# grantjr1842/delayed-streams-modeling

Hardware: AMD Instinct MI355X
Metric: real-time stream throughput, stt-1b-en_fr @ bs=64 per GPU (Mimi encode + LM decode per 80 ms frame) (higher is better)
Workload: dtype bf16 weights + bf16 KV, f32 activations as three exact bf16 pieces, f32 accumulate (v_mfma_f32_16x16x32_bf16); 1 GPU; stt-1b-en_fr batch=64 streaming, ring KV cache full (750 frames), Mimi encode + LM decode HIP path; streams_per_gpu=64, parallelism=replicas x1 (independent stream batches, no per-step collective), streams=encoder stream || 2 LM group stream(s)

## Files before the change

### delayed-streams-modeling_amd/__init__.py

```python
import ctypes as C
import os
import numpy as np

_HERE = os.path.dirname(os.path.abspath(__file__))
LIB_PATH = os.path.join(_HERE, "libdsm_mi355x.so")

FRAME_SIZE = 1920
MAX_RATIOS = 8
MAX_EXTRA_HEADS = 8


class TransformerConfig(C.Structure):
    _fields_ = [(n, C.c_int) for n in (
        "d_model", "num_heads", "num_layers", "dim_feedforward", "context", "max_period",
        "gating", "norm", "positional_embedding", "layer_scale", "conv_layout")]


class MimiConfig(C.Structure):
    _fields_ = [
        ("channels", C.c_int), ("dimension", C.c_int), ("n_filters", C.c_int),
        ("n_residual_layers", C.c_int), ("n_ratios", C.c_int), ("ratios", C.c_int * MAX_RATIOS),
        ("kernel_size", C.c_int), ("residual_kernel_size", C.c_int), ("last_kernel_size", C.c_int),
        ("dilation_base", C.c_int), ("compress", C.c_int), ("transformer", TransformerConfig),
        ("quantizer_n_q", C.c_int), ("quantizer_bins", C.c_int), ("quantizer_dim", C.c_int),
# ... 62 lines not shown
    _fields_ = [("self", C.c_void_p), ("batch_size", C.c_int), ("asr_delay_in_tokens", C.c_int),
                ("extra_heads_num", C.c_int), ("encode_step", BE_ENCODE), ("reset_slot", BE_RESET),
                ("step_tokens", BE_STEP), ("poll_msgs", BE_POLL), ("last_error", BE_ERROR),
                ("encode_async", BE_ENCODE_ASYNC), ("step_ticket", BE_STEP_TICKET)]


class Metrics(C.Structure):
    _fields_ = [("last_encode_us", C.c_double), ("last_lm_us", C.c_double),
                ("algorithmic_bytes_encode", C.c_double), ("algorithmic_bytes_lm", C.c_double),
                ("steps_encode", C.c_uint64), ("steps_lm", C.c_uint64),
                ("graph_launches", C.c_uint64), ("eager_bodies", C.c_uint64),
                ("capture_failures", C.c_uint64), ("capture_error", C.c_char * 96)]


MSG_STEP, MSG_WORD, MSG_END_WORD = 0, 1, 2

ABI_SYMBOLS = [
    "dsm_mimi_config_v0_1", "dsm_asr_config_stt_1b_en_fr", "dsm_asr_config_stt_2_6b_en",
    "dsm_asr_create", "dsm_asr_create_from_arena", "dsm_asr_weight_arena", "dsm_destroy", "dsm_last_error", "dsm_mimi_encode_step", "dsm_asr_step_tokens",
    "dsm_asr_step_pcm", "dsm_asr_poll_msgs", "dsm_asr_reset_slot", "dsm_mimi_reset_slot", "dsm_sync",
    "dsm_get_metrics", "dsm_batch_size", "dsm_n_q", "dsm_mimi_encode_step_dev", "dsm_asr_step_tokens_dev",
    "dsm_streams_join", "dsm_debug_read", "dsm_debug_gemm_plan", "dsm_asr_step_pcm_dev", "dsm_prof_enable", "dsm_prof_read",
    "dsm_asr_create_replica", "dsm_asr_set_seed", "dsm_debug_set_positions", "dsm_debug_set_text_tokens", "dsm_mimi_decode_step", "dsm_mimi_decode_step_dev",
    "dsm_lm_stream_groups", "dsm_debug_serialize_groups", "dsm_prof_read_device", "dsm_prof_timeline", "dsm_prof_timeline_read",
    "dsm_wav_decode", "dsm_mp3_decode", "dsm_mp3_decode_info", "dsm_mp3_probe", "dsm_resample", "dsm_pcm_decode",
    "dsm_mp3_test_synth", "dsm_mp3_test_tables", "dsm_mp3_test_imdct", "dsm_free", "dsm_linear_resampler_new", "dsm_linear_resampler_process",
    "dsm_linear_resampler_free", "dsm_ogg_demux_new", "dsm_ogg_demux_free", "dsm_ogg_demux_push", "dsm_ogg_demux_next",
    "dsm_ogg_demux_info", "dsm_worker_set_opus_decoder", "dsm_ogg_mux_new", "dsm_ogg_mux_free", "dsm_ogg_mux_header", "dsm_ogg_mux_page",
    "dsm_inmsg_encode", "dsm_outmsg_encode", "dsm_inmsg_decode", "dsm_outmsg_decode", "dsm_worker_create",
    "dsm_worker_create_with_backend", "dsm_worker_destroy", "dsm_worker_last_error", "dsm_worker_set_detokenizer", "dsm_worker_open", "dsm_worker_close",
    "dsm_worker_send", "dsm_worker_send_body", "dsm_worker_step", "dsm_worker_step_encode", "dsm_worker_step_model",
    "dsm_mimi_encode_step_async", "dsm_asr_step_tokens_ticket", "dsm_worker_recv", "dsm_worker_buffered",
    "dsm_tts_config_v202501", "dsm_tts_create", "dsm_tts_destroy", "dsm_tts_last_error", "dsm_tts_step",
    "dsm_tts_audio_tokens", "dsm_tts_step_idx", "dsm_tts_reset_slot", "dsm_tts_debug_read", "dsm_tts_get_metrics", "dsm_tts_set_sampling",
    "dsm_tts_set_ca_src", "dsm_tts_attach_mimi", "dsm_tts_step_pcm", "dsm_tts_recv_pcm", "dsm_tts_pcm_pending",
    "dsm_tts_attach_speaker_encoder", "dsm_tts_encode_voice", "dsm_tts_speaker_empty",
]
PROF_TAGS = ["attn_lm", "gemm_lm", "attn_mimi", "gemm_mimi", "rvq", "other"]

_lib = None


def load_library(path=None):
    global _lib
    if _lib is not None and path is None:
        return _lib
    p = path or LIB_PATH
# ... 34 lines not shown
    lib.dsm_mimi_decode_step_dev.argtypes = [vp, vp, vp, vp]
    lib.dsm_mimi_decode_step_dev.restype = C.c_int
    lib.dsm_debug_set_positions.argtypes = [vp, C.c_uint32, C.c_uint32]
    lib.dsm_debug_set_positions.restype = C.c_int
    lib.dsm_asr_create_replica.argtypes = [vp, vp, C.c_int, C.c_int, C.POINTER(vp)]
    lib.dsm_asr_create_replica.restype = C.c_int
    lib.dsm_asr_set_seed.argtypes = [vp, C.c_int, C.c_uint64]
    lib.dsm_asr_set_seed.restype = C.c_int
    lib.dsm_debug_set_text_tokens.argtypes = [vp, vp]
    lib.dsm_debug_set_text_tokens.restype = C.c_int
    lib.dsm_prof_enable.argtypes = [vp, C.c_uint]
    lib.dsm_prof_read.argtypes = [vp, C.POINTER(C.c_double), C.POINTER(C.c_uint64)]
    for name in ("dsm_mimi_encode_step", "dsm_asr_step_tokens", "dsm_asr_step_pcm", "dsm_asr_poll_msgs",
                 "dsm_asr_reset_slot", "dsm_mimi_reset_slot", "dsm_sync", "dsm_get_metrics", "dsm_batch_size",
                 "dsm_n_q", "dsm_mimi_encode_step_dev", "dsm_asr_step_tokens_dev", "dsm_streams_join",
                 "dsm_debug_read", "dsm_asr_step_pcm_dev", "dsm_prof_enable", "dsm_prof_read"):
        getattr(lib, name).restype = C.c_int
    lib.dsm_prof_read_device.argtypes = [vp, C.POINTER(C.c_double), C.POINTER(C.c_uint64)]
    lib.dsm_prof_read_device.restype = C.c_int
    lib.dsm_lm_stream_groups.argtypes = [vp, C.POINTER(C.c_int), C.POINTER(C.c_int), C.c_int]
    lib.dsm_lm_stream_groups.restype = C.c_int
    lib.dsm_debug_serialize_groups.argtypes = [vp, C.c_int]
    lib.dsm_debug_serialize_groups.restype = C.c_int
    lib.dsm_debug_gemm_plan.argtypes = [C.c_int] * 9 + [C.c_char_p, C.c_size_t]
    lib.dsm_debug_gemm_plan.restype = C.c_int
    lib.dsm_wav_decode.argtypes = [C.c_char_p, C.c_size_t, C.POINTER(C.POINTER(C.c_float)), C.POINTER(C.c_size_t),
                                   C.POINTER(C.c_int)]
    lib.dsm_wav_decode.restype = C.c_int
    for name in ("dsm_mp3_decode", "dsm_pcm_decode"):
        getattr(lib, name).argtypes = lib.dsm_wav_decode.argtypes
        getattr(lib, name).restype = C.c_int
    lib.dsm_mp3_decode_info.argtypes = [C.c_char_p, C.c_size_t, C.POINTER(C.POINTER(C.c_float)), C.POINTER(C.c_size_t), C.POINTER(Mp3Info)]
    lib.dsm_mp3_decode_info.restype = C.c_int
    lib.dsm_mp3_probe.argtypes = [C.c_char_p, C.c_size_t, C.POINTER(Mp3Info)]
    lib.dsm_mp3_probe.restype = C.c_int
    lib.dsm_resample.argtypes = [C.c_void_p, C.c_size_t, C.c_int, C.c_int, C.POINTER(C.POINTER(C.c_float)), C.POINTER(C.c_size_t)]
    lib.dsm_resample.restype = C.c_int
    lib.dsm_mp3_test_synth.argtypes = [C.c_void_p, C.c_int, C.c_void_p]
    lib.dsm_mp3_test_tables.argtypes = [C.c_int, C.POINTER(C.c_int), C.POINTER(C.c_int), C.c_void_p, C.c_void_p, C.c_int]
    lib.dsm_mp3_test_imdct.argtypes = [C.c_void_p, C.c_int, C.c_void_p]
    lib.dsm_free.argtypes = [vp]
    lib.dsm_free.restype = None
    lib.dsm_linear_resampler_new.argtypes = [C.c_uint32, C.c_uint32]
    lib.dsm_linear_resampler_new.restype = vp
    lib.dsm_linear_resampler_process.argtypes = [vp, vp, C.c_size_t, vp, C.c_size_t]
    lib.dsm_linear_resampler_process.restype = C.c_size_t
# ... 553 lines not shown
    def prof_read_device(self):
        tot = (C.c_double * len(PROF_TAGS))()
        cnt = (C.c_uint64 * len(PROF_TAGS))()
        self._check(self.lib.dsm_prof_read_device(self.h, tot, cnt))
        return {t: (tot[i], cnt[i]) for i, t in enumerate(PROF_TAGS)}

    def prof_timeline(self, on):
        self._check(self.lib.dsm_prof_timeline(self.h, 1 if on else 0))

    def prof_timeline_read(self, cap=1 << 16):
        sid, kind, tag = (C.c_int * cap)(), (C.c_int * cap)(), (C.c_int * cap)()
        t0, t1 = (C.c_double * cap)(), (C.c_double * cap)()
        n = self._check(self.lib.dsm_prof_timeline_read(self.h, sid, kind, tag, t0, t1, cap))
        return [(sid[i], kind[i], PROF_TAGS[tag[i]], t0[i], t1[i]) for i in range(n)]

    def stream_groups(self):
        a, b = (C.c_int * 8)(), (C.c_int * 8)()
        g = self._check(self.lib.dsm_lm_stream_groups(self.h, a, b, 8))
        return [(a[i], b[i]) for i in range(g)]

    def debug_serialize_groups(self, on):
        self._check(self.lib.dsm_debug_serialize_groups(self.h, 1 if on else 0))

    def prof_enable(self, tags):
        mask = 0
        for t in tags:
            mask |= 1 << PROF_TAGS.index(t)
        self._check(self.lib.dsm_prof_enable(self.h, mask))

    def prof_read(self):
        tot = (C.c_double * len(PROF_TAGS))()
        cnt = (C.c_uint64 * len(PROF_TAGS))()
        self._check(self.lib.dsm_prof_read(self.h, tot, cnt))
        return {t: (tot[i], cnt[i]) for i, t in enumerate(PROF_TAGS)}


class TtsEngine:

    def __init__(self, cfg, batch_size, lm_path, device_id=0):
        self.lib = load_library()
        self.cfg, self.B, self.S = cfg, batch_size, cfg.dep_num_slices
        self.n_speakers = 0
        h = C.c_void_p()
        rc = self.lib.dsm_tts_create(C.byref(cfg), device_id, batch_size, lm_path.encode(), C.byref(h))
        if rc != 0:
            msg = self.lib.dsm_tts_last_error(None)
# ... 104 lines not shown
```

### delayed-streams-modeling_amd/csrc/dsm_engine.hip

```cpp
#include <hip/hip_runtime.h>

#include <cmath>
#include <cstdarg>
#include <cstdio>
#include <cstdlib>
#include <cstring>
#include <atomic>
#include <mutex>
#include <shared_mutex>
#include <string>
#include <set>
#include <vector>

#include "../../include/dsm.h"
#include "dsm_device.h"
#include "dsm_config_presets.h"
#include "dsm_gemm_plan.h"
#include "dsm_kernels.h"
#include "dsm_numerics.h"
#include "dsm_safetensors.h"

static thread_local std::string g_create_error;

static int dsm_env_int(const char* name, int dflt) {
// ... 172 lines not shown
  TransformerState tr;
  struct Group {
    int b0 = 0, nb = 0;
    TransformerState view;
  };
  std::vector<Group> groups;
};

struct HostItem {
  size_t step_idx = 0;
  std::vector<uint32_t> word_tokens;
  bool unended_word = false;
  double last_stop_time = 0.0;
};

}

struct dsm_engine : DsmDevice {
  dsm_asr_config cfg{};
  int B = 0;
  hipEvent_t ev_grp_in[kMaxGroups] = {}, ev_stagger[kMaxGroups] = {};
  bool grp_busy = false;
  bool serialize_groups = false;
  hipEvent_t ev_codes_consumed = nullptr;
  bool codes_consumed_valid = false;
  hipEvent_t ev_join = nullptr, ev_a = nullptr, ev_b = nullptr, ev_c = nullptr, ev_d = nullptr;
  MimiW mimi_w;
  MimiState mimi[2];
  std::atomic<bool> mimi1_ready{false};
  std::mutex mimi1_mu;
  MimiDecState dec;
  LmW lm_w;
  LmState lm;
  GraphSlot *g_enc[2] = {}, *g_grp[kMaxGroups] = {};
  float* h_pcm = nullptr;
  float* h_pcm1 = nullptr;
  uint8_t* h_mask = nullptr;
  uint32_t *h_codes = nullptr, *h_text = nullptr;
  float* h_prs = nullptr;
  std::vector<HostItem> items;
  size_t model_step_idx = 0;
  std::vector<dsm_asr_msg> msgs;
  std::vector<uint32_t> msg_tokens;
  dsm_metrics metrics{};
  static constexpr int kPipe = 4;
  struct PipeSlot {
// ... 534 lines not shown
    case GEMM_BX3_LOOP: hipLaunchKernelGGL((gemm_bx3_kernel<KVT, MT, NT, EPI, true>), grid, block, p.lds, st, a); break;
    case GEMM_BX3_LOOP_NT2:
      if constexpr (MT == 4)
        hipLaunchKernelGGL((gemm_bx3_kernel<KVT, 4, (NT == 1 ? 2 : NT), (EPI == EPI_GATE ? EPI_STORE : EPI), true>), grid, block, p.lds, st, a);
      break;
    case GEMM_BX3_SPLIT:
      if constexpr (MT == 4) hipLaunchKernelGGL((gemm_bx3_kernel<KVT, 4, NT, EPI, false>), grid, block, p.lds, st, a);
      break;
    case GEMM_BX3U_2:
      if constexpr (MT == 2) hipLaunchKernelGGL((gemm_bx3u_kernel<KVT, 2, NT, EPI, 8, 0, 4>), grid, block, p.lds, st, a);
      break;
    case GEMM_BX3U_1:
      if constexpr (MT == 1) hipLaunchKernelGGL((gemm_bx3u_kernel<KVT, 1, NT, EPI, 8>), grid, block, p.lds, st, a);
      break;
    case GEMM_WK:
      if constexpr (MT == 1 && EPI == EPI_GATE && NT == 2)
        hipLaunchKernelGGL((gemm_wk_kernel<KVT, 1, 2, EPI_GATE, 1, 4, 2, true, 4>), grid, block, p.lds, st, a);
      break;
    case GEMM_NO_FIT: break;
  }
}

template <typename WT, typename KVT, int EPI, int NT>
int launch_gemm(DsmDevice* e, hipStream_t st, const GemmArgs& args, bool aligned, Slabs* slabs = nullptr) {
  static_assert(EPI_STORE == GEMM_EPI_STORE && EPI_QKV == GEMM_EPI_QKV && EPI_GATE == GEMM_EPI_GATE && EPI_RVQ == GEMM_EPI_RVQ, "");
  static_assert(LoopDepth<uint16_t, 1>::MAX == 4 && LoopDepth<uint16_t, 2>::MAX == 2 && LoopDepth<float, 1>::MAX == 2, "plan_gemm's `deep`");
  auto ok4 = [](const RowMap& m) { return m.ld % 4 == 0 && m.bstride % 4 == 0; };
  GemmQuery q;
  q.weight_bf16 = sizeof(WT) == 2;
  q.epi = EPI;
  q.NT = NT;
  q.M = args.M; q.N = args.N; q.K = args.K; q.Kpad = args.Kpad;
  q.nt_stride = args.nt_stride;
  q.aligned = aligned;
  q.has_Y = args.Y != nullptr; q.has_Y2 = args.Y2 != nullptr; q.has_res = args.res != nullptr;
  q.has_bias = args.bias != nullptr; q.has_norm = args.norm_out != nullptr;
  q.y_ok4 = ok4(args.ymap); q.y2_ok4 = ok4(args.y2map); q.res_ok4 = ok4(args.rmap);
  q.y_bstride0 = args.ymap.bstride == 0;
  q.may_defer = slabs != nullptr;
  GemmKnobs k;
  k.dot_mode = e->dot_mode;
  k.chunk_loop_min_tiles = e->chunk_loop_min_tiles;
  k.smallk_min_tiles = e->smallk_min_tiles;
  k.smallk_mt = e->smallk_mt;
  k.loop_depth = e->loop_depth;
  const GemmPlan p = plan_gemm(q, k);
  if (p.form == GEMM_NO_FIT) {
    e->set_error("GEMM K=%d: chunk partials do not fit in LDS", args.K);
    return DSM_ERR_INVALID;
  }
  GemmArgs a = args;
  a.vec = p.vec;
  a.chunk_loop = p.chunk_loop;
  a.wg_cols = p.wg_cols;
  a.nt_stride = p.nt_stride;
  a.ws_ntiles = p.ws_ntiles;
  const int sid = e->sid(st);
  if (p.ws_bytes) {
    if (p.ws_bytes > e->gemm_ws_cap[sid]) {
      if (e->capturing) {
        e->capture_failed = true;
        e->set_error("split-K workspace grew during a graph capture");
        return DSM_ERR_STATE;
      }
      e->ws_gen += 1;
      HIPCHK(hipStreamSynchronize(st));
      if (e->gemm_ws[sid]) HIPCHK(hipFree(e->gemm_ws[sid]));
      e->gemm_ws[sid] = nullptr;
      e->gemm_ws_cap[sid] = 0;
      void* ws = nullptr;
      HIPCHK(hipMalloc(&ws, p.ws_bytes));
      e->gemm_ws[sid] = reinterpret_cast<float*>(ws);
      e->gemm_ws_cap[sid] = p.ws_bytes;
    }
    a.ws = e->gemm_ws[sid];
  }
  if (p.tiled) a.ts = e->timeline ? e->dev_ts_slot(e->tag_gemm[sid], sid, 1, 2) : nullptr;
  const int ph = e->prof_begin(e->tag_gemm[sid], st);
  switch (p.MT) {
    case 4: launch_form<WT, KVT, EPI, NT, 4>(p, st, a); break;
    case 2: launch_form<WT, KVT, EPI, NT, 2>(p, st, a); break;
    default: launch_form<WT, KVT, EPI, NT, 1>(p, st, a); break;
  }
  switch (p.reduce) {
    case GEMM_RED_NONE: case GEMM_RED_CONSUMER: break;
    case GEMM_RED_ROWS1: hipLaunchKernelGGL(gemm_reduce_rows_kernel<1>, dim3(a.M), dim3(256), 0, st, a, p.chunks); break;
    case GEMM_RED_ROWS2: hipLaunchKernelGGL(gemm_reduce_rows_kernel<2>, dim3(a.M), dim3(512), 0, st, a, p.chunks); break;
    case GEMM_RED_ROWS4: hipLaunchKernelGGL(gemm_reduce_rows_kernel<4>, dim3(a.M), dim3(1024), 0, st, a, p.chunks); break;
    case GEMM_RED_TILES: {
      const int out_tiles = ((a.M + 15) / 16) * ((a.N + 15) / 16);
      hipLaunchKernelGGL((gemm_reduce_kernel<KVT, EPI>), dim3((out_tiles + 3) / 4), dim3(256), 0, st, a, p.chunks);
      break;
    }
  }
  e->prof_end(ph, st);
  HIPCHK(hipGetLastError());
  if (p.row_norm) {
    hipLaunchKernelGGL(row_norm_kernel, dim3(a.M), dim3(256), 0, st, a.norm_out, a.Y, a.norm_w, a.norm_b, a.M,
                       a.N, a.norm_eps, a.norm_rms);
    HIPCHK(hipGetLastError());
  }
  if (slabs) {
    *slabs = Slabs{};
// ... 90 lines not shown
  a.xmap = xmap;
  a.W = L.w;
  a.wpacked = L.packed ? 1 : 0;
  a.Kpad = L.Kpad;
  a.K = L.K;
  a.N = L.N;
  a.M = M;
  a.nt_stride = 16;
  a.bias = L.bias;
  return a;
}

float norm_eps(int rms) { return rms ? 1e-8f : 1e-5f; }

void set_norm(GemmArgs& a, const float* w, const float* b, float* out, int rms) {
  a.norm_w = w;
  a.norm_b = b;
  a.norm_out = out;
  a.norm_eps = norm_eps(rms);
  a.norm_rms = rms;
}

template <typename WT>
int gemm_store(DsmDevice* e, hipStream_t st, const GemmArgs& a, bool aligned = true, Slabs* slabs = nullptr) {
  return launch_gemm<WT, float, EPI_STORE, 1>(e, st, a, aligned, slabs);
}

int run_conv(DsmDevice* e, hipStream_t st, const ConvGeom& c, const float* cat, int B, float* y, RowMap ymap,
             float* y2, RowMap y2map, const float* res, RowMap rmap) {
  const long bstride = (long)(c.S + c.T_in) * c.in_c;
  GemmArgs a = base_args(c.lin, cat, batch_map(bstride, c.T_out, c.stride * c.in_c, 0), B * c.T_out);
  a.Y = y;
  a.ymap = ymap;
  a.Y2 = y2;
  a.y2map = y2map;
  a.res = res;
  a.rmap = rmap;
  bool aligned = ((c.stride * c.in_c) % 4 == 0) && (bstride % 4 == 0);
  return gemm_store<float>(e, st, a, aligned);
}

}

#include "dsm_engine_api.inc"
#include "dsm_tts.inc"
#include "dsm_speaker.inc"
#include "dsm_audio.inc"
#include "dsm_worker.inc"
```

### delayed-streams-modeling_amd/csrc/dsm_engine_api.inc

```

namespace {

template <typename KVT, int HD, int T>
int launch_attn_t(DsmDevice* e, hipStream_t st, float* out, const float* q, const void* k, const void* v,
                  const uint32_t* start_pos, const uint8_t* active, int B, int H, int ctx, int d, const AttnFused& fq) {
  constexpr int UNR = (sizeof(KVT) == 2 && T == 1 && HD == 128) ? 8 : 4;
  size_t lds = sizeof(float) * ((size_t)T * ctx + 4 * T * HD + 16);
  if ((long)B * H >= 2048 && (size_t)2 * ctx * HD * sizeof(KVT) >= (size_t)256 * 1024) lds += e->attn_lds_pad;
  if (lds > 64 * 1024) {
    static size_t allowed = 0;
    if (lds > allowed) {
      HIPCHK(hipFuncSetAttribute(reinterpret_cast<const void*>(&attn_kernel<KVT, HD, T, UNR>), hipFuncAttributeMaxDynamicSharedMemorySize, (int)lds));
      allowed = lds;
    }
  }
  const int tag = e->tag_attn[e->sid(st)];
  if (T == 1 && HD == 64 && ctx <= 32) {
    const int ph = e->prof_begin(tag, st);
    hipLaunchKernelGGL((attn_small_kernel<KVT, 64>), dim3((B * H + 3) / 4), dim3(256), 0, st, out, q, reinterpret_cast<const KVT*>(k),
                       reinterpret_cast<const KVT*>(v), start_pos, active, B * H, H, ctx, d, fq);
    e->prof_end(ph, st);
    HIPCHK(hipGetLastError());
    return 0;
  }
// ... 132 lines not shown

int fork_groups(DsmDevice* e, hipStream_t st, size_t G) {
  if (G > 1) {
    HIPCHK(hipEventRecord(e->ev_fork, st));
    for (size_t g = 1; g < G; ++g) HIPCHK(hipStreamWaitEvent(e->s_grp[g], e->ev_fork, 0));
  }
  return 0;
}
template <typename F>
int run_groups(DsmDevice* e, hipStream_t st, size_t G, bool serialize, F&& body) {
  for (size_t g = G; g-- > 0;) {
    hipStream_t gs = (g == 0 || serialize) ? st : e->s_grp[g];
    if (int rc = body(g, gs)) return rc;
    if (g > 0) HIPCHK(hipEventRecord(e->ev_grp_done[g], gs));
  }
  return 0;
}
int join_groups(DsmDevice* e, hipStream_t st, size_t G) {
  for (size_t g = 1; g < G; ++g) HIPCHK(hipStreamWaitEvent(st, e->ev_grp_done[g], 0));
  return 0;
}

int seanet_encode(DsmDevice* e, hipStream_t st, const MimiW& w, SeanetEnc& s, const float* cat_init, int B, int r, float* out,
                  RowMap omap, bool front_done = false) {
  const RowMap none = plain_map(1, 1);
  const size_t n = w.stages.size();
  const ConvGeom g0 = over_frames(w.init_conv, r), gf = over_frames(w.final_conv, r);
  if (!front_done)
    if (int rc = run_conv(e, st, g0, cat_init, B, s.stages[0].y, plain_map(B * g0.T_out, g0.out_c), s.stages[0].cat_ra,
                          cat_map(over_frames(w.stages[0].ra, r)), nullptr, none))
      return rc;
  for (size_t i = 0; i < n; ++i) {
    const ConvGeom ra = over_frames(w.stages[i].ra, r), rb = over_frames(w.stages[i].rb, r), dn = over_frames(w.stages[i].down, r);
    SeanetEnc::Stage& ss = s.stages[i];
    if (!(i == 0 && front_done)) {
      if (int rc = run_conv(e, st, ra, ss.cat_ra, B, nullptr, none, ss.cat_rb, cat_map(rb), nullptr, none)) return rc;
      if (int rc = run_conv(e, st, rb, ss.cat_rb, B, nullptr, none, ss.cat_down, cat_map(dn), ss.y, plain_map(B * rb.T_out, rb.out_c)))
        return rc;
    }
    if (i + 1 < n) {
      if (int rc = run_conv(e, st, dn, ss.cat_down, B, s.stages[i + 1].y, plain_map(B * dn.T_out, dn.out_c), s.stages[i + 1].cat_ra,
                            cat_map(over_frames(w.stages[i + 1].ra, r)), nullptr, none))
        return rc;
    } else if (int rc = run_conv(e, st, dn, ss.cat_down, B, nullptr, none, s.cat_final, cat_map(gf), nullptr, none)) {
      return rc;
    }
  }
  return run_conv(e, st, gf, s.cat_final, B, out, omap, nullptr, none, nullptr, none);
}

int mimi_encode_body(dsm_engine* e, int side, hipStream_t st);
int mimi_encode(dsm_engine* e, int side, hipStream_t st) {
  return run_captured(e, *e->g_enc[side], st, (uint64_t)e->sid(st), [&] { return mimi_encode_body(e, side, st); });
}
int mimi_encode_body(dsm_engine* e, int side, hipStream_t st) {
  const MimiW& w = e->mimi_w;
  MimiState& s = e->mimi[side];
  const int B = e->B;
  const RowMap none = plain_map(1, 1);
  e->tag_gemm[e->sid(st)] = DSM_PROF_GEMM_MIMI;
  e->tag_attn[e->sid(st)] = DSM_PROF_ATTN_MIMI;
  bool fused_front = false;
  {
    const MimiW::Stage& s0 = w.stages[0];
    const ConvGeom& c = w.init_conv;
    fused_front = e->fuse_front && c.in_c == 1 && c.k == 7 && c.stride == 1 && c.out_c == 64 && c.S == 6 && !c.lin.bf16 &&
                  s0.ra.k == 3 && s0.ra.stride == 1 && s0.ra.in_c == 64 && s0.ra.out_c == 32 && s0.ra.S == 2 && !s0.ra.lin.bf16 &&
                  s0.rb.k == 1 && s0.rb.stride == 1 && s0.rb.in_c == 32 && s0.rb.out_c == 64 && !s0.rb.lin.bf16 &&
                  c.T_in % 64 == 0 && c.T_out == c.T_in && s0.ra.T_in == c.T_in && s0.rb.T_in == c.T_in && s0.down.in_c == 64 &&
                  s0.down.T_in == c.T_in && !c.replicate && !s0.ra.replicate;
    if (fused_front) {
      SeanetFrontArgs fa;
      fa.cat_init = s.enc.cat_init;
      fa.w0 = reinterpret_cast<const float*>(c.lin.w); fa.b0 = c.lin.bias; fa.ld0 = c.lin.Kpad;
      fa.w1 = reinterpret_cast<const float*>(s0.ra.lin.w); fa.b1 = s0.ra.lin.bias; fa.ld1 = s0.ra.lin.Kpad;
      fa.w2 = reinterpret_cast<const float*>(s0.rb.lin.w); fa.b2 = s0.rb.lin.bias; fa.ld2 = s0.rb.lin.Kpad;
      fa.cat_ra = s.enc.stages[0].cat_ra;
      fa.cat_down = s.enc.stages[0].cat_down;
      fa.T = c.T_in; fa.S0 = c.S; fa.Sd = s0.down.S;
      const int ph = e->prof_begin(e->tag_gemm[e->sid(st)], st);
      hipLaunchKernelGGL(seanet_front_kernel<64>, dim3(c.T_in / 64, B), dim3(256), seanet_front_lds<64>(), st, fa);
      e->prof_end(ph, st);
      HIPCHK(hipGetLastError());
    }
  }
  const int Tt = w.final_conv.T_out, d = w.cfg.dimension;
  if (int rc = seanet_encode(e, st, w, s.enc, s.enc.cat_init, B, 1, s.act.x, plain_map(B * Tt, d), fused_front)) return rc;
  if (int rc = transformer_forward<float, float>(e, st, w.tr, s.tr, s.act, B, Tt, s.mask, s.cat_ds, cat_map(w.downsample))) return rc;
  if (s.first_call && w.downsample.S > 0) {
    hipLaunchKernelGGL(conv_replicate_init_kernel, dim3(B), dim3(256), 0, st, s.h_descs[s.ds_desc]);
    HIPCHK(hipGetLastError());
  }
  if (int rc = run_conv(e, st, w.downsample, s.cat_ds, B, s.latent, plain_map(B, d), nullptr, none, nullptr, none)) return rc;
  const int n_q = w.cfg.quantizer_n_q, qd = w.cfg.quantizer_dim;
  e->tag_gemm[e->sid(st)] = DSM_PROF_RVQ;
  for (int which = 0; which < 2; ++which) {
    const RvqW& r = which == 0 ? w.rvq_first : w.rvq_rest;
    if (r.n_q == 0) continue;
    float* res = which == 0 ? s.res_first : s.res_rest;
    {
      GemmArgs a = base_args(r.input_proj, s.latent, plain_map(B, d), B);
      a.Y = res; a.ymap = plain_map(B, qd);
      if (int rc = gemm_store<float>(e, st, a)) return rc;
    }
    for (int i = 0; i < r.n_q; ++i) {
      const Linear& cb = r.codebooks[i];
      GemmArgs a = base_args(cb, res, plain_map(B, qd), B);
      a.pval = s.pval; a.pidx = s.pidx;
      if (int rc = launch_gemm<float, float, EPI_RVQ, 1>(e, st, a, true)) return rc;
      hipLaunchKernelGGL(rvq_select_kernel, dim3(B), dim3(256), 0, st, s.pval, s.pidx, (cb.N + 15) / 16, B, s.codes, n_q,
// ... 1028 lines not shown
  }
  return 0;
}

int dsm_lm_stream_groups(dsm_engine* e, int* first_slot, int* n_slots, int cap) {
  if (!e) return DSM_ERR_INVALID;
  const int G = (int)e->lm.groups.size();
  for (int g = 0; g < G && g < cap; ++g) {
    if (first_slot) first_slot[g] = e->lm.groups[g].b0;
    if (n_slots) n_slots[g] = e->lm.groups[g].nb;
  }
  return G;
}

int dsm_debug_serialize_groups(dsm_engine* e, int on) {
  if (!e) return DSM_ERR_INVALID;
  HIPCHK(hipSetDevice(e->device));
  ApiShared api(e);
  if (int rc = dsm_sync(e)) return rc;
  e->serialize_groups = on != 0;
  return 0;
}

int dsm_prof_read_device(dsm_engine* e, double* total_us, uint64_t* launches) {
  if (!e) return DSM_ERR_INVALID;
  HIPCHK(hipSetDevice(e->device));
  ApiShared api(e);
  if (int rc = dsm_sync(e)) return rc;
  for (int i = 0; i < DSM_PROF_NTAGS; ++i) {
    if (total_us) total_us[i] = 0;
    if (launches) launches[i] = 0;
  }
  const size_t n = e->dev_ts_tags.size();
  if (n) {
    std::vector<unsigned long long> h(2 * n);
    HIPCHK(hipMemcpy(h.data(), e->dev_ts, sizeof(unsigned long long) * 2 * n, hipMemcpyDeviceToHost));
    int khz = 100000;
    (void)hipDeviceGetAttribute(&khz, hipDeviceAttributeWallClockRate, e->device);
    for (size_t i = 0; i < n; ++i) {
      if (h[2 * i + 1] < h[2 * i]) continue;
      if (total_us) total_us[e->dev_ts_tags[i]] += (double)(h[2 * i + 1] - h[2 * i]) * 1000.0 / khz;
      if (launches) launches[e->dev_ts_tags[i]] += 1;
    }
    for (size_t i = 0; i < n; ++i) { h[2 * i] = ~0ull; h[2 * i + 1] = 0; }
    HIPCHK(hipMemcpy(e->dev_ts, h.data(), sizeof(unsigned long long) * 2 * n, hipMemcpyHostToDevice));
    HIPCHK(hipStreamSynchronize(nullptr));
// ... 84 lines not shown
  else if (nm == "lm.logits") { src = e->lm.logits; n = (size_t)B * e->cfg.text_out_vocab_size; }
  else if (nm == "latent") { src = e->mimi[side].latent; n = (size_t)B * dim; }
  if (!src) { e->set_error("unknown debug tap %s", name); return DSM_ERR_INVALID; }
  if (n > cap) n = cap;
  HIPCHK(hipMemcpy(out, src, sizeof(float) * n, hipMemcpyDeviceToHost));
  return (int)n;
}

int dsm_debug_gemm_plan(int stt, int dot_mode, int weight_bf16, int epi, int nt, int M, int N, int K, int flags, char* buf, size_t cap) {
  if (epi < EPI_STORE || epi > EPI_RVQ || (nt != 1 && nt != 2) || M < 1 || N < 1 || K < 1 || !buf || !cap) return DSM_ERR_INVALID;
  GemmQuery q;
  q.weight_bf16 = weight_bf16 != 0;
  q.epi = epi;
  q.NT = nt;
  q.M = M; q.N = N; q.K = K;
  q.Kpad = round_up(K, 32);
  q.nt_stride = epi == EPI_GATE ? N : 16;
  q.aligned = flags & DSM_GEMMQ_ALIGNED;
  q.has_Y = flags & DSM_GEMMQ_Y; q.has_Y2 = flags & DSM_GEMMQ_Y2; q.has_res = flags & DSM_GEMMQ_RES;
  q.has_bias = flags & DSM_GEMMQ_BIAS; q.has_norm = flags & DSM_GEMMQ_NORM;
  q.y_ok4 = flags & DSM_GEMMQ_Y_OK4; q.y2_ok4 = flags & DSM_GEMMQ_Y2_OK4; q.res_ok4 = flags & DSM_GEMMQ_RES_OK4;
  q.y_bstride0 = flags & DSM_GEMMQ_Y_PLAIN;
  q.may_defer = flags & DSM_GEMMQ_MAY_DEFER;
  return gemm_plan_line(plan_gemm(q, gemm_default_knobs(stt != 0, dot_mode)), q.has_norm, buf, cap);
}

}
```

### delayed-streams-modeling_amd/csrc/dsm_gemm_plan.h

```cpp
#ifndef DSM_GEMM_PLAN_H
#define DSM_GEMM_PLAN_H
#include <stddef.h>
#include <stdio.h>

#include "dsm_numerics.h"

enum { GEMM_EPI_STORE = 0, GEMM_EPI_QKV = 1, GEMM_EPI_GATE = 2, GEMM_EPI_RVQ = 3 };

struct GemmKnobs {
  int dot_mode = 0;
  int chunk_loop_min_tiles = 384;
  int smallk_min_tiles = 1024;
  int smallk_mt = 4;
  int loop_depth = 4;
};
inline GemmKnobs gemm_default_knobs(bool stt, int dot_mode) {
  GemmKnobs k;
  k.dot_mode = dot_mode;
  if (stt && dot_mode == 1) k.chunk_loop_min_tiles = 192;
  return k;
}

struct GemmQuery {
  bool weight_bf16 = false;
  int epi = GEMM_EPI_STORE;
  int NT = 1;
  int M = 0, N = 0, K = 0, Kpad = 0;
  int nt_stride = 16;
  bool aligned = false;
  bool has_Y = false, has_Y2 = false, has_res = false, has_bias = false, has_norm = false;
  bool y_ok4 = false, y2_ok4 = false, res_ok4 = false;
  bool y_bstride0 = false;
  bool may_defer = false;
};

enum GemmForm {
  GEMM_MFMA,
  GEMM_MFMA_BX3,
  GEMM_TILE,
  GEMM_LOOP2,
  GEMM_LOOP_DEEP,
  GEMM_BX3_LOOP,
  GEMM_BX3_LOOP_NT2,
  GEMM_BX3_SPLIT,
  GEMM_BX3U_1,
  GEMM_BX3U_2,
  GEMM_WK,
  GEMM_NO_FIT,
};
enum GemmReduce {
  GEMM_RED_NONE,
  GEMM_RED_CONSUMER,
  GEMM_RED_ROWS1,
  GEMM_RED_ROWS2,
  GEMM_RED_ROWS4,
  GEMM_RED_TILES,
};

struct GemmPlan {
  GemmForm form = GEMM_NO_FIT;
  bool tiled = false;
  bool k_aligned = false;
  int MT = 1;
  unsigned gx = 1, gy = 1, gz = 1, block = 256;
  size_t lds = 0;
  int chunks = 1;
  int chunk_loop = 0;
  int wg_cols = 0, nt_stride = 16, ws_ntiles = 0, vec = 0;
  size_t ws_bytes = 0;
  GemmReduce reduce = GEMM_RED_NONE;
  bool row_norm = false;
};

inline GemmPlan plan_gemm(const GemmQuery& q, const GemmKnobs& k) {
  GemmPlan p;
  const int kchunks = (q.Kpad + DSM_KC - 1) / DSM_KC;
  p.vec = (q.N % 4 == 0) && (!q.has_Y || q.y_ok4) && (!q.has_Y2 || q.y2_ok4) && (!q.has_res || q.res_ok4);
  p.nt_stride = q.nt_stride;

  if (!(q.aligned && q.K % 32 == 0)) {
    const int rounds = (kchunks + 15) / 16;
    const int S = (kchunks + rounds - 1) / rounds;
    const int tiles16 = (q.N + 15) / 16;
    const int nx = (q.epi == GEMM_EPI_GATE) ? tiles16 : (tiles16 + q.NT - 1) / q.NT;
    int MT = (q.NT == 2) ? 2 : 4;
    while (MT > 1 && (q.M <= 16 * (MT / 2) || (long)nx * ((q.M + 16 * MT - 1) / (16 * MT)) * S < 2048 ||
                      (kchunks > 1 && (size_t)kchunks * q.NT * MT * 1024 > 64 * 1024)))
      MT /= 2;
    if (kchunks > 1 && (size_t)kchunks * q.NT * MT * 1024 > 160 * 1024) return p;
    p.form = (k.dot_mode == 1 && q.weight_bf16 && q.epi != GEMM_EPI_RVQ) ? GEMM_MFMA_BX3 : GEMM_MFMA;
    p.k_aligned = q.aligned && (q.K % 32 == 0);
    p.MT = MT;
    p.gx = nx;
    p.gy = (q.M + 16 * MT - 1) / (16 * MT);
    p.block = 64 * S;
    p.lds = kchunks > 1 ? (size_t)kchunks * q.NT * MT * 1024 : 0;
    p.row_norm = q.has_norm;
    return p;
  }

  p.tiled = true;
  int chunks = kchunks;
  const int gx = (q.N + 63) / 64;
  const bool bx3 = k.dot_mode == 1 && q.weight_bf16;
  if (chunks > 1 && (long)gx * ((q.M + 63) / 64) >= k.chunk_loop_min_tiles) {
    p.chunk_loop = chunks;
    chunks = 1;
  }
  if (q.epi == GEMM_EPI_GATE && q.NT == 2) {
    const bool wk_applicable = q.weight_bf16 && k.dot_mode == 1 && q.K % 32 == 0 && q.Kpad == q.K && kchunks <= 4 && q.M <= 64;
    if (wk_applicable && chunks > 1 && q.N % 16 == 0) {
      p.form = GEMM_WK;
      p.gx = q.N / 16;
      p.gz = (q.M + 15) / 16;
      p.lds = (size_t)chunks * 2 * 1024;
      return p;
    }
  }
  int MT = q.M > 32 ? 4 : (q.M > 16 ? 2 : 1);
  while (MT > 1 && (long)gx * chunks * ((q.M + 16 * MT - 1) / (16 * MT)) < 256) MT /= 2;
// ... 62 lines not shown
```

### delayed-streams-modeling_amd/csrc/dsm_kernels.h

```cpp
#pragma once
#include <hip/hip_runtime.h>
#include <stdint.h>
#include "dsm_numerics.h"
#include "dsm_sampling.h"

typedef float f32x4 __attribute__((ext_vector_type(4)));
typedef short dsm_bf16x8 __attribute__((ext_vector_type(8)));

__device__ __forceinline__ float wave_sum64(float v) {
#pragma unroll
  for (int off = 32; off >= 1; off >>= 1) v = v + __shfl_xor(v, off, 64);
  return v;
}

enum { EPI_STORE = 0, EPI_QKV = 1, EPI_GATE = 2, EPI_RVQ = 3 };

struct RowMap {
  long bstride;
  int rpb;
  int ld;
  int toff;
  __host__ __device__ long off(int m) const { return (long)(m / rpb) * bstride + (long)((m % rpb) + toff) * ld; }
};

// ... 501 lines not shown
  }
  launch_stamp_end(a.ts);
}

template <typename WT, int NT>
struct LoopDepth {
  static constexpr int MAX = (NT == 2 || sizeof(WT) == 4) ? 2 : 4;
};
template <typename WT, typename KVT, int MT, int NT, int EPI, int D, int OCC = 2>
__global__ __launch_bounds__(256, OCC) void gemm_loop_kernel(GemmArgs a) {
  static_assert(D == 2 || D == 4, "window depth");
  launch_stamp_begin(a.ts);
  __shared__ __attribute__((aligned(16))) float Xs[2][16 * MT][DSM_XS_LD];
  const int tid = threadIdx.x, lane = tid & 63, wave = tid >> 6;
  const int r = lane & 15, q = lane >> 4;
  const int xu0 = 4 * ((2 * q) ^ dsm_xs_sw(r)), xu1 = xu0 ^ 4;
  const int m_base = blockIdx.z * (16 * MT);
  const int n_base = blockIdx.x * 64 + 16 * wave;
  const WT* W = reinterpret_cast<const WT*>(a.W);
  const WT* wrow[NT];
#pragma unroll
  for (int nt = 0; nt < NT; ++nt) wrow[nt] = dsm_wbase<WT>(a, W, n_base + nt * a.nt_stride, r, q);
  const int wst = dsm_wstep<WT>(a);
  constexpr int PIECES = 16 * MT * 8;
  constexpr bool TWO = PIECES > 256;
  const bool has0 = tid < PIECES;
  const int row0 = has0 ? (tid >> 3) : 0, part = tid & 7;
  int m0 = m_base + row0;
  m0 = m0 < a.M ? m0 : a.M - 1;
  const float* xsrc0 = a.X + a.xmap.off(m0) + 4 * part;
  const int xdst0 = row0 * DSM_XS_LD + 4 * (part ^ dsm_xs_sw(row0));
  int m1 = m_base + row0 + 32;
  m1 = m1 < a.M ? m1 : a.M - 1;
  const float* xsrc1 = a.X + a.xmap.off(m1) + 4 * part;
  const int xdst1 = (row0 + 32) * DSM_XS_LD + 4 * (part ^ dsm_xs_sw(row0));
  const int nb = a.Kpad >> 5;

  f32x4 acc[NT][MT], tot[NT][MT];
#pragma unroll
  for (int nt = 0; nt < NT; ++nt)
#pragma unroll
    for (int mt = 0; mt < MT; ++mt) {
      acc[nt][mt] = (f32x4){0.f, 0.f, 0.f, 0.f};
      tot[nt][mt] = (f32x4){0.f, 0.f, 0.f, 0.f};
    }
  float4 xp0, xp1, xp2, xp3, xq0, xq1, xq2, xq3;
  Raw8<WT> rw0[NT], rw1[NT], rw2[NT], rw3[NT];
#define DSM_LLOAD(S, G)                                                              \
  {                                                                                  \
    const int kb_ = 32 * min((G), nb - 1);                                           \
    xp##S = *reinterpret_cast<const float4*>(xsrc0 + kb_);                           \
    xq##S = TWO ? *reinterpret_cast<const float4*>(xsrc1 + kb_) : xp##S;             \
    _Pragma("unroll") for (int nt = 0; nt < NT; ++nt) rw##S[nt].load(wrow[nt] + (long)kb_ * wst); \
  }
  DSM_LLOAD(0, 0) DSM_LLOAD(1, 1)
  if (D == 4) { DSM_LLOAD(2, 2) DSM_LLOAD(3, 3) }
  __builtin_amdgcn_sched_barrier(0);
  float xbA[MT][8], xbB[MT][8];
#define DSM_LSTORE(S, BUF)                                                           \
  {                                                                                  \
    float* xs_ = &Xs[BUF][0][0];                                                     \
    if (has0) *reinterpret_cast<float4*>(xs_ + xdst0) = xp##S;                       \
    if (TWO) *reinterpret_cast<float4*>(xs_ + xdst1) = xq##S;                        \
  }
#define DSM_LFRAG(XB, BUF)                                                           \
  _Pragma("unroll") for (int mt = 0; mt < MT; ++mt) {                                \
    const float* fp = &Xs[BUF][0][0] + (16 * mt + r) * DSM_XS_LD;                    \
    const float4 f0 = *reinterpret_cast<const float4*>(fp + xu0), f1 = *reinterpret_cast<const float4*>(fp + xu1); \
    XB[mt][0] = f0.x; XB[mt][1] = f0.y; XB[mt][2] = f0.z; XB[mt][3] = f0.w;          \
    XB[mt][4] = f1.x; XB[mt][5] = f1.y; XB[mt][6] = f1.z; XB[mt][7] = f1.w;          \
  }
  DSM_LSTORE(0, 0)
  __syncthreads();
  DSM_LFRAG(xbA, 0)
#define DSM_LMFMA(CUR, S0, S1)                                                       \
  _Pragma("unroll") for (int s = (S0); s < (S1); ++s) {                              \
    _Pragma("unroll") for (int nt = 0; nt < NT; ++nt)                                \
    _Pragma("unroll") for (int mt = 0; mt < MT; ++mt)                                \
      acc[nt][mt] = __builtin_amdgcn_mfma_f32_16x16x4f32(wa[nt][s], CUR[mt][s], acc[nt][mt], 0, 0, 0); \
    if (NT * MT > 1) __builtin_amdgcn_sched_barrier(0);  \
  }
#define DSM_LSTEP(S, SN, CUR, NXT)                                                   \
  {                                                                                  \
    const int gb = g + (S);                                                          \
    float wa[NT][8];                                                                 \
    _Pragma("unroll") for (int nt = 0; nt < NT; ++nt) rw##S[nt].unpack(wa[nt]);      \
// ... 1622 lines not shown
```

### include/dsm.h

```cpp
#ifndef DSM_H
#define DSM_H

#include <stddef.h>
#include <stdint.h>

#ifdef __cplusplus
extern "C" {
#endif

#define DSM_FRAME_SIZE 1920
#define DSM_MAX_RATIOS 8
#define DSM_MAX_EXTRA_HEADS 8

enum {
  DSM_OK = 0,
  DSM_ERR_INVALID = -1,
  DSM_ERR_IO = -2,
  DSM_ERR_DEVICE = -3,
  DSM_ERR_STATE = -4
};

typedef struct dsm_transformer_config {
  int d_model;
  int num_heads;
// ... 152 lines not shown
const char* dsm_tts_last_error(const dsm_tts*);
int dsm_tts_step(dsm_tts*, const uint32_t* prev_text_token, const int32_t* allowed, const uint8_t* mask,
                 uint32_t* text_token_out, uint32_t* audio_out);
int dsm_tts_audio_tokens(dsm_tts*, int slot, int step, uint32_t* out );
int dsm_tts_step_idx(dsm_tts*, int slot);
int dsm_tts_reset_slot(dsm_tts*, int slot);
int dsm_tts_set_sampling(dsm_tts*, int slot, int top_k, float temperature, uint64_t seed);
int dsm_tts_set_ca_src(dsm_tts*, int slot, const float* ca_src, int n, const float* ca_src_uncond, int n_uncond, double cfg_alpha);
int dsm_tts_attach_mimi(dsm_tts*, const dsm_mimi_config* mimi, const char* mimi_safetensors);
int dsm_tts_step_pcm(dsm_tts*, const uint32_t* prev_text_token, const int32_t* allowed, const uint8_t* mask,
                     uint32_t* text_token_out, uint32_t* audio_out,
                     float* pcm_out , uint8_t* pcm_valid_out );
int dsm_tts_recv_pcm(dsm_tts*, float* pcm_out, uint8_t* pcm_valid_out);
int dsm_tts_pcm_pending(dsm_tts*);
int dsm_tts_attach_speaker_encoder(dsm_tts*, int n_speakers, const char* lm_safetensors);
int dsm_tts_encode_voice(dsm_tts*, const float* pcm , int n_clips, int clip_len,
                         float* ca_src_out , int cap_rows, int* rows_out);
int dsm_tts_speaker_empty(dsm_tts*, float* ca_src_out, int cap_rows, int* rows_out);
int dsm_tts_debug_read(dsm_tts*, const char* name, float* out, size_t cap);
int dsm_tts_get_metrics(dsm_tts*, dsm_metrics* out);

int dsm_lm_stream_groups(dsm_engine*, int* first_slot, int* n_slots, int cap);
int dsm_debug_serialize_groups(dsm_engine*, int on);

int dsm_debug_set_positions(dsm_engine*, uint32_t lm_pos, uint32_t mimi_pos);

int dsm_debug_set_text_tokens(dsm_engine*, const uint32_t* tokens);

int dsm_debug_read(dsm_engine*, const char* name, float* out, size_t cap);

enum {
  DSM_GEMMQ_ALIGNED = 1 << 0,
  DSM_GEMMQ_Y = 1 << 1,
  DSM_GEMMQ_Y2 = 1 << 2,
  DSM_GEMMQ_RES = 1 << 3,
  DSM_GEMMQ_BIAS = 1 << 4,
  DSM_GEMMQ_NORM = 1 << 5,
  DSM_GEMMQ_Y_OK4 = 1 << 6,
  DSM_GEMMQ_Y2_OK4 = 1 << 7,
  DSM_GEMMQ_RES_OK4 = 1 << 8,
  DSM_GEMMQ_Y_PLAIN = 1 << 9,
  DSM_GEMMQ_MAY_DEFER = 1 << 10
};
int dsm_debug_gemm_plan(int stt, int dot_mode, int weight_bf16, int epi, int nt, int M, int N, int K, int flags, char* buf, size_t cap);

int dsm_wav_decode(const uint8_t* bytes, size_t len, float** pcm_out, size_t* n_out, int* sample_rate_out);

typedef struct dsm_mp3_info {
  int sample_rate, channels, bitrate_kbps , vbr;
  int frames;
  int info_frames, resyncs, huffman_overruns, frames_without_reservoir;
  uint64_t id3v2_bytes, junk_bytes;
} dsm_mp3_info;
int dsm_mp3_decode(const uint8_t* bytes, size_t len, float** pcm_out, size_t* n_out, int* sample_rate_out);
int dsm_mp3_decode_info(const uint8_t* bytes, size_t len, float** pcm_out, size_t* n_out, dsm_mp3_info* info);
int dsm_mp3_probe(const uint8_t* bytes, size_t len, dsm_mp3_info* out);
int dsm_resample(const float* in, size_t n, int rate_in, int rate_out, float** out, size_t* n_out);
int dsm_pcm_decode(const uint8_t* bytes, size_t len, float** pcm_out, size_t* n_out, int* sample_rate_out);
int dsm_mp3_test_synth(const float* subbands, int slots, float* pcm);
int dsm_mp3_test_tables(int table, int* xlen, int* linbits, uint16_t* codes, uint8_t* lens, int cap);
int dsm_mp3_test_imdct(const float* spectrum, int block_type, float* out);
void dsm_free(void*);
typedef struct dsm_ogg_demux dsm_ogg_demux;
dsm_ogg_demux* dsm_ogg_demux_new(void);
void dsm_ogg_demux_free(dsm_ogg_demux*);
// ... 77 lines not shown
```

Baseline: 1866 x realtime (stream-seconds of audio per wall second).

## Re-plan SEANet conv GEMMs to fill all CUs with smaller M tiles

Adds a fill_chip planning mode for the Mimi encoder's conv GEMMs, on by default. When the default plan launches few workgroups, the planner picks a 32/48/64-row loop tile that spreads work across all 256 CUs, using a simple occupancy cost model. It also adds a 48-row (MT=3) instantiation of the loop kernel, with guarded X staging for partial second pieces. A debug toggle and a graph-capture key bit are added. The risks are smaller tiles reusing weights less, and the cost model's occupancy table being wrong.

```diff
diff --git a/delayed-streams-modeling_amd/__init__.py b/delayed-streams-modeling_amd/__init__.py
--- a/delayed-streams-modeling_amd/__init__.py
+++ b/delayed-streams-modeling_amd/__init__.py
@@ -108,7 +108,7 @@
     "dsm_get_metrics", "dsm_batch_size", "dsm_n_q", "dsm_mimi_encode_step_dev", "dsm_asr_step_tokens_dev",
     "dsm_streams_join", "dsm_debug_read", "dsm_debug_gemm_plan", "dsm_asr_step_pcm_dev", "dsm_prof_enable", "dsm_prof_read",
     "dsm_asr_create_replica", "dsm_asr_set_seed", "dsm_debug_set_positions", "dsm_debug_set_text_tokens", "dsm_mimi_decode_step", "dsm_mimi_decode_step_dev",
-    "dsm_lm_stream_groups", "dsm_debug_serialize_groups", "dsm_prof_read_device", "dsm_prof_timeline", "dsm_prof_timeline_read",
+    "dsm_lm_stream_groups", "dsm_debug_serialize_groups", "dsm_debug_conv_fill", "dsm_prof_read_device", "dsm_prof_timeline", "dsm_prof_timeline_read",
     "dsm_wav_decode", "dsm_mp3_decode", "dsm_mp3_decode_info", "dsm_mp3_probe", "dsm_resample", "dsm_pcm_decode",
     "dsm_mp3_test_synth", "dsm_mp3_test_tables", "dsm_mp3_test_imdct", "dsm_free", "dsm_linear_resampler_new", "dsm_linear_resampler_process",
     "dsm_linear_resampler_free", "dsm_ogg_demux_new", "dsm_ogg_demux_free", "dsm_ogg_demux_push", "dsm_ogg_demux_next",
@@ -189,6 +189,8 @@
     lib.dsm_lm_stream_groups.restype = C.c_int
     lib.dsm_debug_serialize_groups.argtypes = [vp, C.c_int]
     lib.dsm_debug_serialize_groups.restype = C.c_int
+    lib.dsm_debug_conv_fill.argtypes = [vp, C.c_int]
+    lib.dsm_debug_conv_fill.restype = C.c_int
     lib.dsm_debug_gemm_plan.argtypes = [C.c_int] * 9 + [C.c_char_p, C.c_size_t]
     lib.dsm_debug_gemm_plan.restype = C.c_int
     lib.dsm_wav_decode.argtypes = [C.c_char_p, C.c_size_t, C.POINTER(C.POINTER(C.c_float)), C.POINTER(C.c_size_t),
@@ -788,6 +790,9 @@
     def debug_serialize_groups(self, on):
         self._check(self.lib.dsm_debug_serialize_groups(self.h, 1 if on else 0))
 
+    def debug_conv_fill(self, on):
+        self._check(self.lib.dsm_debug_conv_fill(self.h, 1 if on else 0))
+
     def prof_enable(self, tags):
         mask = 0
         for t in tags:
diff --git a/delayed-streams-modeling_amd/csrc/dsm_engine.hip b/delayed-streams-modeling_amd/csrc/dsm_engine.hip
--- a/delayed-streams-modeling_amd/csrc/dsm_engine.hip
+++ b/delayed-streams-modeling_amd/csrc/dsm_engine.hip
@@ -218,6 +218,7 @@
   hipEvent_t ev_grp_in[kMaxGroups] = {}, ev_stagger[kMaxGroups] = {};
   bool grp_busy = false;
   bool serialize_groups = false;
+  bool conv_fill = true;
   hipEvent_t ev_codes_consumed = nullptr;
   bool codes_consumed_valid = false;
   hipEvent_t ev_join = nullptr, ev_a = nullptr, ev_b = nullptr, ev_c = nullptr, ev_d = nullptr;
@@ -798,7 +799,7 @@
 }
 
 template <typename WT, typename KVT, int EPI, int NT>
-int launch_gemm(DsmDevice* e, hipStream_t st, const GemmArgs& args, bool aligned, Slabs* slabs = nullptr) {
+int launch_gemm(DsmDevice* e, hipStream_t st, const GemmArgs& args, bool aligned, Slabs* slabs = nullptr, bool fill_chip = false) {
   static_assert(EPI_STORE == GEMM_EPI_STORE && EPI_QKV == GEMM_EPI_QKV && EPI_GATE == GEMM_EPI_GATE && EPI_RVQ == GEMM_EPI_RVQ, "");
   static_assert(LoopDepth<uint16_t, 1>::MAX == 4 && LoopDepth<uint16_t, 2>::MAX == 2 && LoopDepth<float, 1>::MAX == 2, "plan_gemm's `deep`");
   auto ok4 = [](const RowMap& m) { return m.ld % 4 == 0 && m.bstride % 4 == 0; };
@@ -814,6 +815,7 @@
   q.y_ok4 = ok4(args.ymap); q.y2_ok4 = ok4(args.y2map); q.res_ok4 = ok4(args.rmap);
   q.y_bstride0 = args.ymap.bstride == 0;
   q.may_defer = slabs != nullptr;
+  q.fill_chip = fill_chip;
   GemmKnobs k;
   k.dot_mode = e->dot_mode;
   k.chunk_loop_min_tiles = e->chunk_loop_min_tiles;
@@ -855,6 +857,16 @@
   const int ph = e->prof_begin(e->tag_gemm[sid], st);
   switch (p.MT) {
     case 4: launch_form<WT, KVT, EPI, NT, 4>(p, st, a); break;
+    case 3:
+      if constexpr (sizeof(WT) == 4 && EPI == EPI_STORE && NT == 1) {
+        if (p.form == GEMM_LOOP2) {
+          hipLaunchKernelGGL((gemm_loop_kernel<WT, KVT, 3, NT, EPI, 2>), dim3(p.gx, p.gy, p.gz), dim3(p.block), p.lds, st, a);
+          break;
+        }
+      }
+      e->prof_end(ph, st);
+      e->set_error("GEMM plan asks for 48-row tiles on a form that has none");
+      return DSM_ERR_INVALID;
     case 2: launch_form<WT, KVT, EPI, NT, 2>(p, st, a); break;
     default: launch_form<WT, KVT, EPI, NT, 1>(p, st, a); break;
   }
@@ -991,12 +1003,12 @@
 }
 
 template <typename WT>
-int gemm_store(DsmDevice* e, hipStream_t st, const GemmArgs& a, bool aligned = true, Slabs* slabs = nullptr) {
-  return launch_gemm<WT, float, EPI_STORE, 1>(e, st, a, aligned, slabs);
+int gemm_store(DsmDevice* e, hipStream_t st, const GemmArgs& a, bool aligned = true, Slabs* slabs = nullptr, bool fill_chip = false) {
+  return launch_gemm<WT, float, EPI_STORE, 1>(e, st, a, aligned, slabs, fill_chip);
 }
 
 int run_conv(DsmDevice* e, hipStream_t st, const ConvGeom& c, const float* cat, int B, float* y, RowMap ymap,
-             float* y2, RowMap y2map, const float* res, RowMap rmap) {
+             float* y2, RowMap y2map, const float* res, RowMap rmap, bool fill_chip = false) {
   const long bstride = (long)(c.S + c.T_in) * c.in_c;
   GemmArgs a = base_args(c.lin, cat, batch_map(bstride, c.T_out, c.stride * c.in_c, 0), B * c.T_out);
   a.Y = y;
@@ -1006,7 +1018,7 @@
   a.res = res;
   a.rmap = rmap;
   bool aligned = ((c.stride * c.in_c) % 4 == 0) && (bstride % 4 == 0);
-  return gemm_store<float>(e, st, a, aligned);
+  return gemm_store<float>(e, st, a, aligned, nullptr, fill_chip);
 }
 
 }
diff --git a/delayed-streams-modeling_amd/csrc/dsm_engine_api.inc b/delayed-streams-modeling_amd/csrc/dsm_engine_api.inc
--- a/delayed-streams-modeling_amd/csrc/dsm_engine_api.inc
+++ b/delayed-streams-modeling_amd/csrc/dsm_engine_api.inc
@@ -178,36 +178,37 @@
 }
 
 int seanet_encode(DsmDevice* e, hipStream_t st, const MimiW& w, SeanetEnc& s, const float* cat_init, int B, int r, float* out,
-                  RowMap omap, bool front_done = false) {
+                  RowMap omap, bool front_done = false, bool fill_chip = false) {
   const RowMap none = plain_map(1, 1);
   const size_t n = w.stages.size();
   const ConvGeom g0 = over_frames(w.init_conv, r), gf = over_frames(w.final_conv, r);
   if (!front_done)
     if (int rc = run_conv(e, st, g0, cat_init, B, s.stages[0].y, plain_map(B * g0.T_out, g0.out_c), s.stages[0].cat_ra,
-                          cat_map(over_frames(w.stages[0].ra, r)), nullptr, none))
+                          cat_map(over_frames(w.stages[0].ra, r)), nullptr, none, fill_chip))
       return rc;
   for (size_t i = 0; i < n; ++i) {
     const ConvGeom ra = over_frames(w.stages[i].ra, r), rb = over_frames(w.stages[i].rb, r), dn = over_frames(w.stages[i].down, r);
     SeanetEnc::Stage& ss = s.stages[i];
     if (!(i == 0 && front_done)) {
-      if (int rc = run_conv(e, st, ra, ss.cat_ra, B, nullptr, none, ss.cat_rb, cat_map(rb), nullptr, none)) return rc;
-      if (int rc = run_conv(e, st, rb, ss.cat_rb, B, nullptr, none, ss.cat_down, cat_map(dn), ss.y, plain_map(B * rb.T_out, rb.out_c)))
+      if (int rc = run_conv(e, st, ra, ss.cat_ra, B, nullptr, none, ss.cat_rb, cat_map(rb), nullptr, none, fill_chip)) return rc;
+      if (int rc = run_conv(e, st, rb, ss.cat_rb, B, nullptr, none, ss.cat_down, cat_map(dn), ss.y, plain_map(B * rb.T_out, rb.out_c), fill_chip))
         return rc;
     }
     if (i + 1 < n) {
       if (int rc = run_conv(e, st, dn, ss.cat_down, B, s.stages[i + 1].y, plain_map(B * dn.T_out, dn.out_c), s.stages[i + 1].cat_ra,
-                            cat_map(over_frames(w.stages[i + 1].ra, r)), nullptr, none))
+                            cat_map(over_frames(w.stages[i + 1].ra, r)), nullptr, none, fill_chip))
         return rc;
-    } else if (int rc = run_conv(e, st, dn, ss.cat_down, B, nullptr, none, s.cat_final, cat_map(gf), nullptr, none)) {
+    } else if (int rc = run_conv(e, st, dn, ss.cat_down, B, nullptr, none, s.cat_final, cat_map(gf), nullptr, none, fill_chip)) {
       return rc;
     }
   }
-  return run_conv(e, st, gf, s.cat_final, B, out, omap, nullptr, none, nullptr, none);
+  return run_conv(e, st, gf, s.cat_final, B, out, omap, nullptr, none, nullptr, none, fill_chip);
 }
 
 int mimi_encode_body(dsm_engine* e, int side, hipStream_t st);
 int mimi_encode(dsm_engine* e, int side, hipStream_t st) {
-  return run_captured(e, *e->g_enc[side], st, (uint64_t)e->sid(st), [&] { return mimi_encode_body(e, side, st); });
+  return run_captured(e, *e->g_enc[side], st, (uint64_t)e->sid(st) | ((uint64_t)e->conv_fill << 32),
+                      [&] { return mimi_encode_body(e, side, st); });
 }
 int mimi_encode_body(dsm_engine* e, int side, hipStream_t st) {
   const MimiW& w = e->mimi_w;
@@ -241,7 +242,7 @@
     }
   }
   const int Tt = w.final_conv.T_out, d = w.cfg.dimension;
-  if (int rc = seanet_encode(e, st, w, s.enc, s.enc.cat_init, B, 1, s.act.x, plain_map(B * Tt, d), fused_front)) return rc;
+  if (int rc = seanet_encode(e, st, w, s.enc, s.enc.cat_init, B, 1, s.act.x, plain_map(B * Tt, d), fused_front, e->conv_fill)) return rc;
   if (int rc = transformer_forward<float, float>(e, st, w.tr, s.tr, s.act, B, Tt, s.mask, s.cat_ds, cat_map(w.downsample))) return rc;
   if (s.first_call && w.downsample.S > 0) {
     hipLaunchKernelGGL(conv_replicate_init_kernel, dim3(B), dim3(256), 0, st, s.h_descs[s.ds_desc]);
@@ -1316,6 +1317,15 @@
   return 0;
 }
 
+int dsm_debug_conv_fill(dsm_engine* e, int on) {
+  if (!e) return DSM_ERR_INVALID;
+  HIPCHK(hipSetDevice(e->device));
+  ApiShared api(e);
+  if (int rc = dsm_sync(e)) return rc;
+  e->conv_fill = on != 0;
+  return 0;
+}
+
 int dsm_prof_read_device(dsm_engine* e, double* total_us, uint64_t* launches) {
   if (!e) return DSM_ERR_INVALID;
   HIPCHK(hipSetDevice(e->device));
@@ -1446,6 +1456,7 @@
   q.y_ok4 = flags & DSM_GEMMQ_Y_OK4; q.y2_ok4 = flags & DSM_GEMMQ_Y2_OK4; q.res_ok4 = flags & DSM_GEMMQ_RES_OK4;
   q.y_bstride0 = flags & DSM_GEMMQ_Y_PLAIN;
   q.may_defer = flags & DSM_GEMMQ_MAY_DEFER;
+  q.fill_chip = flags & DSM_GEMMQ_FILL_CHIP;
   return gemm_plan_line(plan_gemm(q, gemm_default_knobs(stt != 0, dot_mode)), q.has_norm, buf, cap);
 }
 
diff --git a/delayed-streams-modeling_amd/csrc/dsm_gemm_plan.h b/delayed-streams-modeling_amd/csrc/dsm_gemm_plan.h
--- a/delayed-streams-modeling_amd/csrc/dsm_gemm_plan.h
+++ b/delayed-streams-modeling_amd/csrc/dsm_gemm_plan.h
@@ -32,6 +32,7 @@
   bool y_ok4 = false, y2_ok4 = false, res_ok4 = false;
   bool y_bstride0 = false;
   bool may_defer = false;
+  bool fill_chip = false;
 };
 
 enum GemmForm {
@@ -71,6 +72,13 @@
   GemmReduce reduce = GEMM_RED_NONE;
   bool row_norm = false;
 };
+
+enum { GEMM_CUS = 256 };
+inline int gemm_fill_occ(bool loop, int MT) {
+  static const int occ_loop[5] = {0, 6, 4, 4, 3}, occ_tile[5] = {0, 3, 3, 0, 2};
+  return loop ? occ_loop[MT] : occ_tile[MT];
+}
+inline long gemm_fill_cost(long wgs, int occ, int MT) { return (wgs + (long)GEMM_CUS * occ - 1) / ((long)GEMM_CUS * occ) * MT; }
 
 inline GemmPlan plan_gemm(const GemmQuery& q, const GemmKnobs& k) {
   GemmPlan p;
@@ -96,6 +104,32 @@
     p.block = 64 * S;
     p.lds = kchunks > 1 ? (size_t)kchunks * q.NT * MT * 1024 : 0;
     p.row_norm = q.has_norm;
+    return p;
+  }
+
+  if (q.fill_chip && !q.weight_bf16 && q.epi == GEMM_EPI_STORE && q.NT == 1 && q.N > 64 && !q.has_norm && !q.may_defer) {
+    GemmQuery q0 = q;
+    q0.fill_chip = false;
+    const GemmPlan t = plan_gemm(q0, k);
+    const long t_wgs = (long)t.gx * t.gy * t.gz;
+    const int t_occ = gemm_fill_occ(t.form == GEMM_LOOP2, t.MT);
+    if (t.chunks > 1 || t_wgs > 2L * GEMM_CUS * t_occ) return t;
+    const long gx0 = (q.N + 63) / 64;
+    int best = 0;
+    long best_cost = 0, best_wgs = 0;
+    const long t_load = (t_wgs + GEMM_CUS - 1) / GEMM_CUS * t.MT;
+    const bool t_whole_k = t.form == GEMM_LOOP2, t_one_round = t_wgs <= (long)GEMM_CUS * t_occ;
+    for (int mt = 2; mt <= 4; ++mt) {
+      const long wgs = gx0 * ((q.M + 16 * mt - 1) / (16 * mt)), cost = gemm_fill_cost(wgs, gemm_fill_occ(true, mt), mt);
+      if (t_whole_k && t_one_round && (wgs + GEMM_CUS - 1) / GEMM_CUS * mt >= t_load) continue;
+      if (!best || cost <= best_cost) { best = mt; best_cost = cost; best_wgs = wgs; }
+    }
+    if (!best || best_wgs < GEMM_CUS || best_cost > gemm_fill_cost(t_wgs, t_occ, t.MT) || (t_whole_k && t.MT == best)) return t;
+    p = t;
+    p.form = GEMM_LOOP2;
+    p.MT = best;
+    p.chunk_loop = kchunks > 1 ? kchunks : 0;
+    p.gz = (q.M + 16 * best - 1) / (16 * best);
     return p;
   }
 
diff --git a/delayed-streams-modeling_amd/csrc/dsm_kernels.h b/delayed-streams-modeling_amd/csrc/dsm_kernels.h
--- a/delayed-streams-modeling_amd/csrc/dsm_kernels.h
+++ b/delayed-streams-modeling_amd/csrc/dsm_kernels.h
@@ -547,15 +547,17 @@
 #pragma unroll
   for (int nt = 0; nt < NT; ++nt) wrow[nt] = dsm_wbase<WT>(a, W, n_base + nt * a.nt_stride, r, q);
   const int wst = dsm_wstep<WT>(a);
+  static_assert(MT >= 1 && MT <= 4, "two pieces per thread stage at most 64 rows");
   constexpr int PIECES = 16 * MT * 8;
   constexpr bool TWO = PIECES > 256;
   const bool has0 = tid < PIECES;
+  const bool has1 = PIECES >= 512 || tid + 256 < PIECES;
   const int row0 = has0 ? (tid >> 3) : 0, part = tid & 7;
   int m0 = m_base + row0;
   m0 = m0 < a.M ? m0 : a.M - 1;
   const float* xsrc0 = a.X + a.xmap.off(m0) + 4 * part;
   const int xdst0 = row0 * DSM_XS_LD + 4 * (part ^ dsm_xs_sw(row0));
-  int m1 = m_base + row0 + 32;
+  int m1 = m_base + (has1 ? row0 + 32 : 0);
   m1 = m1 < a.M ? m1 : a.M - 1;
   const float* xsrc1 = a.X + a.xmap.off(m1) + 4 * part;
   const int xdst1 = (row0 + 32) * DSM_XS_LD + 4 * (part ^ dsm_xs_sw(row0));
@@ -586,7 +588,7 @@
   {                                                                                  \
     float* xs_ = &Xs[BUF][0][0];                                                     \
     if (has0) *reinterpret_cast<float4*>(xs_ + xdst0) = xp##S;                       \
-    if (TWO) *reinterpret_cast<float4*>(xs_ + xdst1) = xq##S;                        \
+    if (TWO && has1) *reinterpret_cast<float4*>(xs_ + xdst1) = xq##S;                \
   }
 #define DSM_LFRAG(XB, BUF)                                                           \
   _Pragma("unroll") for (int mt = 0; mt < MT; ++mt) {                                \
diff --git a/include/dsm.h b/include/dsm.h
--- a/include/dsm.h
+++ b/include/dsm.h
@@ -198,6 +198,7 @@
 
 int dsm_lm_stream_groups(dsm_engine*, int* first_slot, int* n_slots, int cap);
 int dsm_debug_serialize_groups(dsm_engine*, int on);
+int dsm_debug_conv_fill(dsm_engine*, int on);
 
 int dsm_debug_set_positions(dsm_engine*, uint32_t lm_pos, uint32_t mimi_pos);
 
@@ -216,7 +217,8 @@
   DSM_GEMMQ_Y2_OK4 = 1 << 7,
   DSM_GEMMQ_RES_OK4 = 1 << 8,
   DSM_GEMMQ_Y_PLAIN = 1 << 9,
-  DSM_GEMMQ_MAY_DEFER = 1 << 10
+  DSM_GEMMQ_MAY_DEFER = 1 << 10,
+  DSM_GEMMQ_FILL_CHIP = 1 << 11
 };
 int dsm_debug_gemm_plan(int stt, int dot_mode, int weight_bf16, int epi, int nt, int M, int N, int K, int flags, char* buf, size_t cap);
 
```

Measured after the change: 1877 x realtime (stream-seconds of audio per wall second) (median of 6 runs). About the same (+0.6%).
